# paninski-lab/lightning-pose

Hardware: AMD Instinct MI355X
Metric: training frames/sec (whole node), ResNet-50 384x384 17-kp semi-sup (higher is better)
Workload: dtype bf16; 1 GPU; C2/C3: ResNet-50 SemiSupervisedHeatmapTracker 384x384, K=17, 64 labeled + 128 unlabeled frames per GPU, heatmap_mse + temporal + pca_singleview + unimodal_mse, Adam (backbone lr=0 as at step 0), bf16-mixed; global_batch=192, parallelism=dp1, sync_batchnorm=False, decode_prune=plain kernels (chosen from the maps)

## Files before the change

### include/lp_hip.h

```cpp
#ifndef LP_HIP_H
#define LP_HIP_H

#include <stddef.h>
#include <stdint.h>

#ifdef __cplusplus
extern "C" {
#endif

typedef void* lp_stream_t;

int lp_config_reload_env(void);

enum {
    LP_OK = 0,
    LP_ERR_ARGUMENT = -1,
    LP_ERR_UNSUPPORTED = -2,
};

enum { LP_TF_NONE = 0, LP_TF_SINGLE = 1, LP_TF_PER_FRAME = 2, LP_TF_PER_VIEW = 3 };

#define LP_HIP_ABI_VERSION 153
int lp_version(void);
const char* lp_strerror(int code);


typedef struct lp_decode_tables {
    const int* row_base;
    const float* row_taps;
    const int* col_start;
    const float* col_taps;
    const int* colT_start;
    const float* colT_taps;
    int ty, tx, tc;
} lp_decode_tables;

typedef struct lp_frame_map {
// ... 80 lines not shown
    int B, Hi, Wi, Ci;
    int Ho, Wo, Co;
    int R, S, stride, pad;
} lp_conv_geom;

#define LP_CONV_KERNEL_IGEMM 0
#define LP_CONV_KERNEL_PIPE 1
#define LP_CONV_KERNEL_WGRAD 2
#define LP_CONV_KERNEL_WGRAD_PIPE 3
#define LP_CONV_KERNEL_PIPE_HALO 4
#define LP_CONV_KERNEL_STEM_WGRAD_NB 8
#define LP_CONV_KERNEL_WGRAD_NB 9
#define LP_CONV_KERNEL_RES2D 5
int lp_conv_last_kernel(void);
int lp_conv_last_resident(void);

int lp_conv_fwd(const void* x, const void* w, const lp_conv_geom* geom, const float* bias, void* out_bf16, float* out_f32, int ldo,
                int n_store, lp_stream_t stream);
int lp_conv_dgrad(const void* dy, const void* wd, const lp_conv_geom* geom, const float* bias, const void* addend,
                  const void* relu_mask, void* dx_bf16, float* dx_f32, int ldo, int n_store, int skip_empty_classes,
                  lp_stream_t stream);
typedef struct lp_gemm_batch {
    int nb, nh;
    long long a_b, a_h, b_b, b_h, c_b, c_h;
} lp_gemm_batch;
int lp_gemm_nt(const void* a, int lda, const void* b, int ldb, void* c_bf16, float* c_f32, int ldc, int M, int N, int K, int n_store,
               const float* bias, const lp_gemm_batch* batch, lp_stream_t stream);
int lp_gemm_tn(const void* x, int ldx, const void* y, int ldy, void* out_bf16, int ldo, int M, int J, int N, const lp_gemm_batch* batch,
               lp_stream_t stream);
int lp_attn_fwd(const void* qkv_bf16, int ld_qkv, int k_off, int v_off, int B, int nh, int T, float scale, void* p_bf16, int ldp,
// ... 304 lines not shown
```

### lightning-pose_amd/_lib.py

```python

from __future__ import annotations

import ctypes as C
import os

_HERE = os.path.dirname(os.path.abspath(__file__))
LIB_PATH = os.environ.get("LP_HIP_LIB") or os.path.join(_HERE, "liblp_hip.so")


class LpHipUnavailable(RuntimeError):
    """liblp_hip.so could not be loaded, or an op was given a non-ROCm tensor.  There is no fallback path."""


class LpHipError(RuntimeError):
    pass


class DecodeTables(C.Structure):
    _fields_ = [("row_base", C.c_void_p), ("row_taps", C.c_void_p), ("col_start", C.c_void_p),
                ("col_taps", C.c_void_p), ("colT_start", C.c_void_p), ("colT_taps", C.c_void_p),
                ("ty", C.c_int), ("tx", C.c_int), ("tc", C.c_int)]


class FrameMap(C.Structure):
# ... 34 lines not shown
CONV_KERNEL_LABEL = {
    CONV_KERNEL_PIPE: (("conv_igemm_kernel", "conv_pipe_kernel"),),
    CONV_KERNEL_PIPE_HALO: (("conv_igemm_kernel", "conv_pipe_kernel"), (">", ",halo>")),
    CONV_KERNEL_RES2D: (("conv_igemm_kernel<64,", "conv_res2d_kernel<"), ("conv_igemm_kernel<64>", "conv_res2d_kernel<fwd>")),
    CONV_KERNEL_WGRAD_PIPE: (("conv_wgrad_kernel", "conv_wgrad_pipe_kernel"),),
    CONV_KERNEL_WGRAD_NB: (("conv_wgrad_kernel", "conv_wgrad_nb_kernel"),),
}
BORDER_RENORM, BORDER_CLAMP = 0, 1
AUG_GEOM, AUG_BLUR, AUG_DROPOUT, AUG_DROP_PER_CHANNEL, AUG_SALT, AUG_PEPPER = 1, 2, 4, 8, 16, 32
AUG_ELASTIC, AUG_HISTEQ, AUG_CLAHE, AUG_EMBOSS, AUG_CROPPAD, AUG_HFLIP = 64, 128, 256, 512, 1024, 2048
AUG_OP_DROPOUT, AUG_OP_SALT, AUG_OP_PEPPER, AUG_OP_ELASTIC = 0, 1, 2, 3
AUG_LOCAL_BLUR_COARSE, AUG_LOCAL_EMBOSS = 0, 1
AUG_ELASTIC_MAX_RADIUS = 20
TF_NONE, TF_SINGLE, TF_PER_FRAME, TF_PER_VIEW = 0, 1, 2, 3

ABI_VERSION = 153

_P, _I, _F, _L, _Z = C.c_void_p, C.c_int, C.c_float, C.c_long, C.c_size_t

PROTOTYPES = {
    "lp_version": (_I, []),
    "lp_strerror": (C.c_char_p, [_I]),
    "lp_config_reload_env": (_I, []),
    "lp_decode_window": (_I, [_I, _I]),
    "lp_decode_fwd": (_I, [_P, _I, _I, _I, _I, _I, _F, C.POINTER(DecodeTables), C.POINTER(FrameMap), _P, _P, _P, _P, _I, _P]),
    "lp_decode_bwd": (_I, [_P, _I, _I, _I, _I, _I, _F, C.POINTER(DecodeTables), C.POINTER(FrameMap), _P, _P, _P, _P, _I, _I, _P]),
    "lp_frame_map_apply": (_I, [_P, _I, _I, C.POINTER(FrameMap), _I, _P, _P]),
    "lp_heatmap_gen": (_I, [_P, _P, _I, _I, _I, _I, _I, _I, _F, _P, _P]),
    "lp_heatmap_gen_bwd": (_I, [_P, _P, _I, _I, _I, _I, _I, _I, _F, _P, _P, _P]),
    "lp_temporal_heatmap_workspace_bytes": (_Z, [_I, _I]),
    "lp_temporal_heatmap_fwd": (_I, [_I, _P, _P, _I, _I, _I, _I, _P, _F, _P, _P, _P]),
# ... 16 lines not shown
    "lp_kp_metrics": (_I, [_P, _P, _I, _I, C.POINTER(PcaSpec), C.POINTER(PcaSpec), _P, _P, _P, _P, _P]),
    "lp_conv_fwd": (_I, [_P, _P, C.POINTER(ConvGeom), _P, _P, _P, _I, _I, _P]),
    "lp_conv_dgrad": (_I, [_P, _P, C.POINTER(ConvGeom), _P, _P, _P, _P, _P, _I, _I, _I, _P]),
    "lp_conv_dgrad_bits": (_I, [_P, _P, C.POINTER(ConvGeom), _P, _P, _P, _I, _P]),
    "lp_gemm_nt": (_I, [_P, _I, _P, _I, _P, _P, _I, _I, _I, _I, _I, _P, C.POINTER(GemmBatch), _P]),
    "lp_gemm_nt_gelu_bwd": (_I, [_P, _P, _P, _P, _I, _I, _I, _P, _P]),
    "lp_gemm_nt_gelu_fwd": (_I, [_P, _P, _P, _P, _P, _I, _I, _I, _P]),
    "lp_gemm_tn": (_I, [_P, _I, _P, _I, _P, _I, _I, _I, _I, C.POINTER(GemmBatch), _P]),
    "lp_attn_fwd": (_I, [_P, _I, _I, _I, _I, _I, _I, C.c_float, _P, _I, _P, _I, _P]),
    "lp_attn_bwd_kv": (_I, [_P, _I, _I, _P, _I, _P, _I, _P, _I, _I, _I, C.c_float, _P, _P, _I, _I, _I, _P]),
    "lp_attn_rowdot": (_I, [_P, _P, _I, _I, _I, _P, _P]),
    "lp_attn_dscores": (_I, [_P, _I, _P, _I, _P, _P, _I, C.c_longlong, C.c_longlong, C.c_float, _P, _I, _I, _I, _I, C.POINTER(GemmBatch), _P]),
    "lp_conv_fwd_bn": (_I, [_P, _P, C.POINTER(ConvGeom), _P, C.POINTER(BnFuse), _P]),
    "lp_conv_last_kernel": (_I, []),
    "lp_conv_last_resident": (_I, []),
    "lp_stem_fwd_bn": (_I, [_P, _P, C.POINTER(ConvGeom), _P, C.POINTER(BnFuse), _P]),
    "lp_conv_dgrad_bn": (_I, [_P, _P, C.POINTER(ConvGeom), _P, _P, _P, C.POINTER(BnFuse), _P]),
    "lp_bn_fold": (_I, [_P, _P, _P, _P, _P, _F, _I, _I, _P, _P, _P]),
    "lp_conv_fwd_act": (_I, [_P, _P, C.POINTER(ConvGeom), _P, _P, _I, _P, _P]),
    "lp_conv_wgrad_workspace_bytes": (_Z, [C.POINTER(ConvGeom), _I]),
    "lp_conv_wgrad": (_I, [_P, _P, C.POINTER(ConvGeom), _P, _I, _P, _Z, _P]),
    "lp_conv_wgrad_bias": (_I, [_P, _P, C.POINTER(ConvGeom), _P, _P, _I, _P, C.c_size_t, _P]),
    "lp_stem_fwd": (_I, [_P, _P, C.POINTER(ConvGeom), _P, _P]),
    "lp_stem_wgrad": (_I, [_P, _P, C.POINTER(ConvGeom), _P, _I, _P, _Z, _P]),
    "lp_bn_reduce_workspace_bytes": (_Z, [_I, _I]),
    "lp_bn_stats": (_I, [_P, _I, _I, _P, _P, _Z, _P]),
    "lp_bn_finalize": (_I, [_P, _F, _I, _F, _F, _P, _P, _P, _P, _P]),
    "lp_fxsum_accumulate": (_I, [_P, _I, _P, _P]),
    "lp_bn_finalize_f32": (_I, [_P, _F, _I, _F, _F, _P, _P, _P, _P, _P]),
    "lp_bn_finalize2": (_I, [_P, _F, _F, _I, _F, _F, _P, _P, _P, _P, _P]),
# ... 156 lines not shown
```

### lightning-pose_amd/csrc/api.hip

```cpp
#include "lp_common.h"

#include <stdlib.h>

#include <atomic>

extern "C" int lp_version(void) { return LP_HIP_ABI_VERSION; }

namespace lp {
static int env_int(const char* name, int dflt) {
    const char* e = getenv(name);
    return (e == nullptr || *e == 0) ? dflt : atoi(e);
}
static LpSwitches read_switches() {
    LpSwitches s;
    s.conv_pipe = env_int("LP_CONV_PIPE", 1);
    s.conv_halo = env_int("LP_CONV_HALO", 1);
    s.pipe_wres = env_int("LP_PIPE_WRES", 1);
    s.conv_res2d = env_int("LP_CONV_RES2D", 1);
    s.infer_pipe = env_int("LP_INFER_PIPE", 1);
    s.gemm_pipe = env_int("LP_GEMM_PIPE", 1);
    s.wgrad_pipe = env_int("LP_WGRAD_PIPE", 1);
    s.wgrad_nb = env_int("LP_WGRAD_NB", 1);
    s.stem_2d = env_int("LP_STEM_2D", 1);
    s.stem_wgrad_nb = env_int("LP_STEM_WGRAD_NB", 1);
    s.pool_v2 = env_int("LP_POOL_V2", 1);
    s.bn_bwd_wgs_per_cu = env_int("LP_BN_BWD_WGS_PER_CU", 5);
    if (s.bn_bwd_wgs_per_cu < 1 || s.bn_bwd_wgs_per_cu > 5) s.bn_bwd_wgs_per_cu = 5;
    s.conv_max_wgs = env_int("LP_CONV_MAX_WGS", 0);
    return s;
}
static std::atomic<const LpSwitches*> g_switches{new LpSwitches(read_switches())};
const LpSwitches& lp_switches() { return *g_switches.load(std::memory_order_acquire); }
}

extern "C" int lp_config_reload_env(void) {
    lp::g_switches.store(new lp::LpSwitches(lp::read_switches()), std::memory_order_release);
    return LP_OK;
// ... 10 lines not shown
```

### lightning-pose_amd/csrc/conv.hip

```cpp
#include <stdlib.h>

#include "lp_common.h"

namespace lp {

constexpr int kBM = 128;
constexpr int kBK = 64;
constexpr int kLD = kBK + 8;

struct ConvGeom {
    int B, Hi, Wi, Ci;
    int Ho, Wo, Co;
    int R, S, stride, pad;
};

struct ConvEpilogue {
    unsigned short* out_bf16;
    float* out_f32;
    int ldo;
    int n_store;
    const float* bias;
    const unsigned short* addend;
    const unsigned short* relu_mask;
    const unsigned char* relu_bits;
// ... 908 lines not shown
}

static long long seg_split_rows(int seg_images, int B, long long rows_per_image, long long M) {
    if (seg_images <= 0) return M;
    if (seg_images >= B) return -1;
    const long long r = (long long)seg_images * rows_per_image;
    return (r % kBM == 0) ? r : -1;
}

static void bn_fuse_begin(ConvEpilogue& ep, const lp_bn_fuse* bn) {
    ep.stats_sums = bn->sums;
    ep.seg_images = bn->seg_images;
}

static thread_local int g_last_conv_kernel = LP_CONV_KERNEL_IGEMM;
static thread_local int g_last_conv_resident = 0;

struct ConvRoute {
    int kernel;
    int bn;
    int mode;
    int ek;
    bool wres;
};
constexpr int kNoKernel = -1;

struct ConvProblem {
    int mode;
    int ek;
    const void *x, *w;
// ... 231 lines not shown
    const long long b_elems = (z.nb - 1) * z.b_b + (z.nh - 1) * z.b_h + (long long)(N - 1) * ldb + K;
    const long long c_elems = (z.nb - 1) * z.c_b + (z.nh - 1) * z.c_h + (long long)M * ldc;
    if (a_elems >= (1LL << 31) || b_elems >= (1LL << 31) || c_elems >= (1LL << 32)) return LP_ERR_UNSUPPORTED;
    if ((z.a_b | z.a_h | z.b_b | z.b_h) % 8 != 0 || (z.c_b | z.c_h) % c_align != 0) return LP_ERR_UNSUPPORTED;
    p = conv_problem(mode, a, b, ConvGeom{1, 1, M, K, 1, M, N, 1, 1, 1, 0}, 1, M, N, K);
    p.dense = z.nb * z.nh == 1 && lda == K && ldb == K && ldc == N;
    p.gemm = true, p.nz = z.nb * z.nh, p.x_bytes = (unsigned)(2 * a_elems), p.w_bytes = (unsigned)(2 * b_elems);
    p.gx = GemmExt{lda, ldb, z.nh, 0, (unsigned)(2 * z.a_b), (unsigned)(2 * z.a_h), (unsigned)(2 * z.b_b), (unsigned)(2 * z.b_h), (unsigned)z.c_b,
                   (unsigned)z.c_h};
    return LP_OK;
}

}
#include "conv_stem_wgrad.h"
#include "conv_wgrad_nb.h"
namespace lp {

constexpr int kWgradWgs = 512;

struct WgradRoute {
    bool ok;
    int kernel;
    int split, per;
    size_t ws_floats;
    int bn, tiles_a, tiles_b;
    bool swap, tuned;
    int Ka, Cb;
    int kh, PT, lead;
};

static void slice_pixels(WgradRoute& p, int units, int ksteps, int split, int cap) {
    if (split > cap) split = cap;
    if (split < 1) split = 1;
    p.per = ((ksteps + split - 1) / split) * kBK;
    p.split = (units + p.per - 1) / p.per;
}

static WgradRoute plan_wgrad(int M, int Kw, int Co, int split_hint) {
    WgradRoute p{};
    p.kernel = LP_CONV_KERNEL_WGRAD;
    p.bn = Co > 64 ? 128 : 64;
    p.tiles_a = (Kw + kBM - 1) / kBM;
    p.tiles_b = p.bn == 128 ? (Co + 127) / 128 : 1;
    const int tiles = p.tiles_a * p.tiles_b, ksteps = (M + kBK - 1) / kBK;
    slice_pixels(p, M, ksteps, split_hint > 0 ? split_hint : kWgradWgs / tiles, ksteps < 65535 ? ksteps : 65535);
    p.ws_floats = (size_t)p.split * tiles * 4 * 2 * (p.bn / 64) * 16 * 64;
    p.ok = true;
    return p;
}

// ... 32 lines not shown
    if (split <= 0) {
        double best = 1e30;
        for (int s = 1; s <= 2 * cus && s <= ksteps / 2; ++s) {
            if (s != 1 && (tiles * s) % cus > 0 && (tiles * (s + 1) + cus - 1) / cus == (tiles * s + cus - 1) / cus) continue;
            const double rounds = (double)((tiles * s + cus - 1) / cus), per = (double)((ksteps + s - 1) / s);
            const double cost = rounds * per + 0.04 * (p.bn / 128.0) * s * tiles + 2.0 * rounds;
            if (cost < best) best = cost, split = s;
        }
    }
    slice_pixels(p, M, ksteps, split, ksteps / 2);
    p.ws_floats = (size_t)p.split * tiles * 256 * p.bn;
    p.ok = true;
    return p;
}

static WgradRoute plan_wgrad_nb(const ConvGeom& g, int split_hint) {
    WgradRoute p{};
    if (g.R != 3 || g.S != 3 || g.stride != 1 || g.pad != 1 || g.Hi != g.Ho || g.Wi != g.Wo || g.Ci % 64 != 0 || g.Co % 64 != 0) return p;
    if (g.Wi > 126) return p;
    const long long pt = (long long)g.B * (g.Hi + 1) * (g.Wi + 1);
    if (pt + 64 * 8 >= (1LL << 31)) return p;
    p.kernel = LP_CONV_KERNEL_WGRAD_NB;
    p.PT = (int)pt;
    p.lead = 1 + (g.Wi + 1) / 64;
    p.bn = g.Co % 128 == 0 ? 128 : 64;
    p.kh = p.bn == 64 ? 2 : 1;
    p.tiles_a = g.Ci / 64;
    p.tiles_b = g.Co / p.bn;
    const int tiles = p.tiles_a * p.tiles_b;
    const int ksteps = (p.PT + kBK - 1) / kBK;
// ... 6 lines not shown
            const double rounds = (double)((tiles * s + cus - 1) / cus), per = (double)((ksteps + s - 1) / s);
            const double cost = rounds * (per * step_us + 15.0) + 0.06 * s * tiles;
            if (cost < best) best = cost, split = s;
        }
    }
    slice_pixels(p, p.PT, ksteps, split, ksteps < 65535 ? ksteps : 65535);
    p.ws_floats = (size_t)p.split * p.kh * tiles * 9 * 64 * p.bn;
    p.ok = true;
    return p;
}

static bool is_stem(const ConvGeom& g) { return g.R == 7 && g.S == 7 && g.stride == 2 && g.pad == 3 && g.Ci == 4 && g.Co == 64; }

struct WgradCandidates {
    int n;
    WgradRoute r[3];
};

static WgradCandidates wgrad_candidates(const ConvGeom& g, bool stem, int split_hint) {
    WgradCandidates c{};
    const int M = g.B * g.Ho * g.Wo;
    auto add = [&c](const WgradRoute& p) {
        if (p.ok) c.r[c.n++] = p;
    };
    if (stem) {
        if (lp_switches().stem_wgrad_nb != 0) add(plan_stem_wgrad_nb(g, split_hint));
        add(plan_wgrad(M, 256, 64, split_hint));
    } else {
        add(plan_wgrad_nb(g, split_hint));
        add(plan_wgrad_pipe(g, split_hint));
        add(plan_wgrad(M, g.R * g.S * g.Ci, g.Co, split_hint));
    }
    return c;
}

static const WgradRoute& route_wgrad(const WgradCandidates& c, const LpSwitches& sw, bool dbias) {
    const bool pipe = !dbias && sw.conv_pipe != 0;
    for (int i = 0; i < c.n - 1; ++i) {
        const WgradRoute& r = c.r[i];
        if (r.kernel == LP_CONV_KERNEL_WGRAD_NB && !(pipe && sw.wgrad_pipe == 1 && sw.wgrad_nb != 0)) continue;
        if (r.kernel == LP_CONV_KERNEL_WGRAD_PIPE && !(pipe && sw.wgrad_pipe != 0 && (sw.wgrad_pipe == 2 || r.tuned))) continue;
        return r;
    }
    return c.r[c.n - 1];
}

template <int BN>
static void launch_wgrad(const WgradRoute& p, const void* x, const void* dy, const ConvGeom& g, float* dw, float* dbias, float* ws, hipStream_t st) {
    const int M = g.B * g.Ho * g.Wo, Kw = g.R * g.S * g.Ci, tiles = p.tiles_a * p.tiles_b;
    const unsigned x_bytes = (unsigned)(2ull * g.B * g.Hi * g.Wi * g.Ci), dy_bytes = (unsigned)(2ull * M * g.Co);
    TnExt ext{};
    ext.col_sums = dbias;
    const auto kernel = dbias ? conv_wgrad_kernel<BN, false, true> : conv_wgrad_kernel<BN, false, false>;
    hipLaunchKernelGGL(kernel, dim3(tiles * p.split), dim3(256), 0, st, (const unsigned short*)x, (const unsigned short*)dy, x_bytes, dy_bytes, g,
                       M, Kw, tiles, p.tiles_b, p.per, make_fastdiv(g.Ho * g.Wo), make_fastdiv(g.Wo), ws, ext);
    launch_wgrad_reduce<BN>(ws, p.split, tiles, p.tiles_b, Kw, g.Co, dw, st);
// ... 7 lines not shown
    const void *pa = x, *qb = dy;
    unsigned pa_bytes = x_bytes, qb_bytes = dy_bytes;
    if (p.swap) {
        wg = WgradPipeGeom{g.B, g.Ho, g.Wo, g.Ho, g.Wo, g.Co, 1, 1, 1, 0, p.Ka, p.Cb, 1};
        pa = dy, qb = x, pa_bytes = dy_bytes, qb_bytes = x_bytes;
    } else {
        const int plain = g.R == 1 && g.S == 1 && g.stride == 1 && g.pad == 0 && g.Hi == g.Ho && g.Wi == g.Wo;
        wg = WgradPipeGeom{g.B, g.Hi, g.Wi, g.Ho, g.Wo, g.Ci, g.R, g.S, g.stride, g.pad, p.Ka, p.Cb, plain};
    }
    const int tiles = p.tiles_a * p.tiles_b;
    const int sa = p.swap ? Kw : 1, sb = p.swap ? 1 : Kw;
    hipLaunchKernelGGL((conv_wgrad_pipe_kernel<BN>), dim3(tiles * p.split), dim3(512), 0, st, (const unsigned short*)pa, (const unsigned short*)qb,
                       pa_bytes, qb_bytes, wg, M, tiles, p.tiles_b, p.per, make_fastdiv(g.Ho * g.Wo), make_fastdiv(g.Wo), ws);
    hipLaunchKernelGGL((wgrad_pipe_reduce_kernel<BN>), dim3(tiles * 256 * BN / 64), dim3(256), 0, st, ws, p.split, tiles, p.tiles_b, p.Ka, p.Cb,
                       sa, sb, dw);
}

template <int BN>
static void launch_wgrad_nb(const WgradRoute& p, const void* x, const void* dy, const ConvGeom& g, float* dw, float* ws, hipStream_t st) {
    const unsigned x_bytes = (unsigned)(2ull * g.B * g.Hi * g.Wi * g.Ci), dy_bytes = (unsigned)(2ull * g.B * g.Ho * g.Wo * g.Co);
    const WgradNbGeom ng{g.B, g.Hi, g.Wi, g.Ci, g.Co, p.PT, p.lead};
    const int tiles = p.tiles_a * p.tiles_b;
    hipLaunchKernelGGL((conv_wgrad_nb_kernel<BN>), dim3(tiles * p.split), dim3(512), 0, st, (const unsigned short*)x, (const unsigned short*)dy,
                       x_bytes, dy_bytes, ng, tiles, p.tiles_b, p.per, make_fastdiv(g.Wi + 1), make_fastdiv(g.Hi + 1), ws);
    hipLaunchKernelGGL((wgrad_nb_reduce_kernel<BN>), dim3(tiles * 9 * BN), dim3(256), 0, st, ws, p.split * p.kh, tiles, p.tiles_b, g.Ci, dw);
}

static bool geom_ok(const lp_conv_geom* c) {
    return c && c->B > 0 && c->Hi > 0 && c->Wi > 0 && c->Ci > 0 && c->Ho > 0 && c->Wo > 0 && c->Co > 0 && c->R > 0 && c->S > 0 &&
           c->stride > 0 && c->pad >= 0;
// ... 17 lines not shown
    ConvProblem p = conv_problem(kModeFwd, x, w, g, g.Ho, g.Wo, g.Co, g.R * g.S * g.Ci);
    p.ek = kEkNone;
    p.ep = ConvEpilogue{(unsigned short*)out_bf16, out_f32, ldo, n_store > 0 ? n_store : p.N, bias};
    if (bn) {
        LP_REQUIRE(bn->sums && bn->seg_images >= 0);
        if (p.N % 8 != 0) return LP_ERR_UNSUPPORTED;
        p.seg_rows = seg_split_rows(bn->seg_images, g.B, (long long)g.Ho * g.Wo, p.M);
        if (p.seg_rows < 0) return LP_ERR_UNSUPPORTED;
        bn_fuse_begin(p.ep, bn);
    }
    return run_conv(p, stream);
}

extern "C" int lp_conv_last_kernel(void) { return lp::g_last_conv_kernel; }
extern "C" int lp_conv_last_resident(void) { return lp::g_last_conv_resident; }

extern "C" int lp_conv_fwd(const void* x, const void* w, const lp_conv_geom* geom, const float* bias, void* out_bf16, float* out_f32,
                           int ldo, int n_store, lp_stream_t stream) {
    return conv_fwd_impl(x, w, geom, bias, out_bf16, out_f32, ldo, n_store, nullptr, stream);
}

extern "C" int lp_conv_fwd_act(const void* x, const void* w, const lp_conv_geom* geom, const float* bias, const void* residual_bf16, int relu,
                               void* out_bf16, lp_stream_t stream) {
    using namespace lp;
    LP_REQUIRE(x && w && geom_ok(geom) && out_bf16);
    ConvGeom g = to_geom(geom);
    if (g.Ci % kBK != 0 || g.Co % 8 != 0 || g.R * g.S > 32 || (long long)g.B * g.Hi * g.Wi * g.Ci >= (1LL << 31) ||
        (long long)g.B * g.Ho * g.Wo * g.Co >= (1LL << 32))
        return LP_ERR_UNSUPPORTED;
    ConvProblem p = conv_problem(kModeInfer, x, w, g, g.Ho, g.Wo, g.Co, g.R * g.S * g.Ci);
// ... 175 lines not shown
static int conv_wgrad_impl(const void* x, const void* dy, const lp_conv_geom* geom, float* dw, float* dbias, int split_hint, void* workspace,
                           size_t workspace_bytes, lp_stream_t stream) {
    using namespace lp;
    LP_REQUIRE(x && dy && geom_ok(geom) && dw && workspace);
    ConvGeom g = to_geom(geom);
    if (g.Ci % 8 != 0 || g.Co % 8 != 0 || (long long)g.B * g.Hi * g.Wi * g.Ci >= (1LL << 31) ||
        (long long)g.B * g.Ho * g.Wo * g.Co >= (1LL << 31))
        return LP_ERR_UNSUPPORTED;
    const WgradCandidates c = wgrad_candidates(g, false, split_hint);
    const WgradRoute& p = route_wgrad(c, lp_switches(), dbias != nullptr);
    LP_REQUIRE(workspace_bytes >= p.ws_floats * sizeof(float));
    hipStream_t st = (hipStream_t)stream;
    float* ws = (float*)workspace;
    g_last_conv_kernel = p.kernel;
    g_last_conv_resident = 0;
    if (p.kernel == LP_CONV_KERNEL_WGRAD_NB) {
        if (p.bn == 128) launch_wgrad_nb<128>(p, x, dy, g, dw, ws, st);
        else launch_wgrad_nb<64>(p, x, dy, g, dw, ws, st);
    } else if (p.kernel == LP_CONV_KERNEL_WGRAD_PIPE) {
        if (p.bn == 128) launch_wgrad_pipe<128>(p, x, dy, g, dw, ws, st);
        else launch_wgrad_pipe<64>(p, x, dy, g, dw, ws, st);
    } else {
        if (p.bn == 128) launch_wgrad<128>(p, x, dy, g, dw, dbias, ws, st);
        else launch_wgrad<64>(p, x, dy, g, dw, dbias, ws, st);
    }
    return launch_status();
}

extern "C" int lp_conv_wgrad(const void* x, const void* dy, const lp_conv_geom* geom, float* dw, int split_hint, void* workspace,
                             size_t workspace_bytes, lp_stream_t stream) {
    return conv_wgrad_impl(x, dy, geom, dw, nullptr, split_hint, workspace, workspace_bytes, stream);
}

extern "C" int lp_conv_wgrad_bias(const void* x, const void* dy, const lp_conv_geom* geom, float* dw, float* dbias, int split_hint,
                                  void* workspace, size_t workspace_bytes, lp_stream_t stream) {
// ... 68 lines not shown
                             size_t workspace_bytes, lp_stream_t stream) {
    using namespace lp;
    LP_REQUIRE(x4 && dy && geom_ok(geom) && dw && workspace);
    ConvGeom g = to_geom(geom);
    if (!is_stem(g)) return LP_ERR_UNSUPPORTED;
    const WgradCandidates c = wgrad_candidates(g, true, split_hint);
    const WgradRoute& p = route_wgrad(c, lp_switches(), false);
    LP_REQUIRE(workspace_bytes >= p.ws_floats * sizeof(float));
    const int M = g.B * g.Ho * g.Wo, Kw = 256;
    const unsigned short *xs = (const unsigned short*)x4, *dys = (const unsigned short*)dy;
    const FastDiv dhw = make_fastdiv(g.Ho * g.Wo), dwo = make_fastdiv(g.Wo);
    hipStream_t st = (hipStream_t)stream;
    float* ws = (float*)workspace;
    g_last_conv_kernel = p.kernel;
    g_last_conv_resident = 0;
    if (p.kernel == LP_CONV_KERNEL_STEM_WGRAD_NB)
        hipLaunchKernelGGL(stem_wgrad_nb_kernel, dim3(p.split), dim3(256), 0, st, xs, dys, (unsigned)(8ull * g.B * g.Hi * g.Wi),
                           (unsigned)(128ull * M), g, M, p.per, dhw, dwo, ws);
    else
        hipLaunchKernelGGL((conv_wgrad_kernel<64, true>), dim3(p.tiles_a * p.split), dim3(256), 0, st, xs, dys, 0u, 0u, g, M, Kw, p.tiles_a, 1,
                           p.per, dhw, dwo, ws, TnExt{});
    launch_wgrad_reduce<64>(ws, p.split, p.tiles_a, 1, Kw, 64, dw, st);
    return launch_status();
}
```

### lightning-pose_amd/csrc/lp_common.h

```cpp
#pragma once

#include <hip/hip_runtime.h>
#include <stdint.h>

#include "../../include/lp_hip.h"

namespace lp {

constexpr int kWave = 64;

typedef __attribute__((ext_vector_type(8))) __bf16 bf16x8;
typedef __attribute__((ext_vector_type(8))) unsigned short u16x8;
typedef __attribute__((ext_vector_type(4))) unsigned short u16x4;
typedef __attribute__((ext_vector_type(4))) float f32x4;
typedef __attribute__((ext_vector_type(16))) float f32x16;

__device__ __forceinline__ float bf16_to_f32(unsigned short b) { return __uint_as_float(((unsigned)b) << 16); }

#if defined(__HIP_DEVICE_COMPILE__)
typedef __attribute__((ext_vector_type(2))) __bf16 bf16x2_t;
typedef __attribute__((ext_vector_type(2))) float f32x2_t;
__device__ __forceinline__ unsigned short f32_to_bf16(float f) { return __builtin_bit_cast(unsigned short, (__bf16)f); }
__device__ __forceinline__ unsigned pack_bf16x2(float lo, float hi) {
    const f32x2_t v = {lo, hi};
// ... 232 lines not shown
    }
    td = fmin(fmax(td, -0x1p49), 0x1p49);
    const double h = rint(td * 0x1p12);
    const long long hi = (long long)h;
    const long long lo = (long long)rint((td - h * 0x1p-12) * 0x1p60);
    atomicAdd(reinterpret_cast<unsigned long long*>(&p->hi), (unsigned long long)hi);
    atomicAdd(reinterpret_cast<unsigned long long*>(&p->lo), (unsigned long long)lo);
}
__device__ __forceinline__ float fx_value(const lp_fxsum* p) {
    const long long lo = p->lo;
    if (lo >= kFxPoisonSeen || lo <= -kFxPoisonSeen) return __int_as_float(0x7fc00000);
    return (float)((double)p->hi * 0x1p-12 + (double)lo * 0x1p-60);
}

struct LpSwitches {
    int conv_pipe, conv_halo, pipe_wres, conv_res2d, infer_pipe, gemm_pipe, wgrad_pipe, wgrad_nb, stem_2d, stem_wgrad_nb, pool_v2, conv_max_wgs, bn_bwd_wgs_per_cu;
};
const LpSwitches& lp_switches();

inline int launch_status() {
    hipError_t e = hipGetLastError();
    return e == hipSuccess ? LP_OK : (int)e;
}

}

#define LP_REQUIRE(cond)                    \
    do {                                    \
        if (!(cond)) return LP_ERR_ARGUMENT; \
    } while (0)
```

### lightning-pose_amd/engine.py

```python

from __future__ import annotations

import ctypes as C
import math
import os
from dataclasses import dataclass, field

import torch
import torch.distributed as dist

from . import _lib
from ._lib import check
from . import ops
from .ops import _p

BN_EPS = 1e-5
BN_MOMENTUM = 0.1
CPAD = 64


@dataclass
class ConvP:
    name: str
    kind: str
# ... 227 lines not shown
        return torch.zeros(n, device=self.device, dtype=torch.float32)

    def _zeros_fx(self, n: int) -> torch.Tensor:
        return self._zeros_f32(4 * n).view(torch.int64)

    def _timed(self, tag: str, flops: float, fn, nbytes: float = 0.0, layer: str = ""):
        if self.profile is None:
            return fn()
        e0, e1 = torch.cuda.Event(enable_timing=True), torch.cuda.Event(enable_timing=True)
        e0.record()
        out = fn()
        e1.record()
        if tag.startswith("conv_") and hasattr(self._lib, "lp_conv_last_kernel"):
            for old, new in _lib.CONV_KERNEL_LABEL.get(self._lib.lp_conv_last_kernel(), ()):
                tag = tag.replace(old, new)
        self.profile.append((tag, flops, e0, e1, nbytes, layer))
        return out

    def _wgrad(self, x, dy, g, dw: torch.Tensor, stem: bool = False, dbias: torch.Tensor | None = None) -> None:
        need = self._lib.lp_conv_wgrad_workspace_bytes(C.byref(g), 0)
        if self._wgrad_ws is None or self._wgrad_ws.numel() < need:
            self._join_side_stream()
            self._wgrad_ws = torch.empty(max(need, 96 << 20), device=self.device, dtype=torch.uint8)
        fn = self._lib.lp_stem_wgrad if stem else self._lib.lp_conv_wgrad
        what = "lp_stem_wgrad" if stem else "lp_conv_wgrad"
        if dbias is not None:
            what = "lp_conv_wgrad_bias"
            fn = lambda x_, dy_, g_, dw_, split, ws, nws, st: self._lib.lp_conv_wgrad_bias(x_, dy_, g_, dw_, _p(dbias), split, ws, nws, st)
        if self.device.type != "cuda" or not self.wgrad_side_stream or self.profile is not None:
            check(fn(_p(x), _p(dy), C.byref(g), _p(dw), 0, _p(self._wgrad_ws), self._wgrad_ws.numel(), ops._stream()), what)
# ... 709 lines not shown
```

### profiles/kernel_resources.py

```python
import os
import re
import shutil
import subprocess
import sys
import tempfile

ROOT = os.path.dirname(os.path.dirname(os.path.abspath(__file__)))
LLVM = os.path.join(os.environ.get("ROCM_PATH", "/opt/rocm"), "lib", "llvm", "bin")
HOT = ("lp::conv_pipe_kernel", "lp::conv_spec_kernel", "lp::conv_wgrad_pipe_kernel", "lp::conv_res2d_kernel", "lp::conv_stem2d_kernel", "lp::conv_wgrad_kernel", "lp::stem_wgrad_nb_kernel", "lp::conv_wgrad_nb_kernel",
       "lp::conv_igemm_kernel", "lp::bn_apply_kernel", "lp::bn_bwd_apply_kernel", "lp::bn_relu_maxpool_fwd_kernel", "lp::bn_pool_bwd_v2_kernel",
       "lp::colreduce_kernel", "lp::rows_reduce_kernel", "lp::decode_fwd_kernel", "lp::decode_bwd_kernel", "lp::heatmap_gen_kernel",
       "lp::hm_rowsq_kernel", "lp::hm_grad_kernel", "lp::softmax2d", "lp::adam_kernel", "lp::pca_kernel", "lp::temporal_kernel",
       "lp::attn_fwd_kernel", "lp::attn_bwd_kv_kernel", "lp::pixel_shuffle",
       "lp::layernorm_ls_fwd_kernel", "lp::layernorm_ls_bwd_kernel",
       "lp::rope_kernel", "lp::vit_reg_tokens_fwd_kernel", "lp::vit_reg_tokens_bwd_kernel",
       "lp::window_partition_kernel", "lp::window_unpartition_kernel", "lp::vit_pos_tokens_fwd_kernel", "lp::vit_pos_tokens_bwd_kernel",
       "lp::resid_out_fwd_kernel", "lp::resid_out_bwd_kernel",
       "lp::frames_crop_resize_kernel", "lp::bbox_from_keypoints_kernel", "lp::bbox_smooth_kernel")
ALLOWED_SCRATCH = (
    re.compile(r"lp::decode_bwd_kernel<\d+, \d+, 64, "),
    re.compile(r"lp::bn_bwd_apply_kernel<false, false>"),
    re.compile(r"lp::conv_igemm_kernel<128, 1>"),
)

# ... 48 lines not shown
```

Measured before the change: 4851 frames/s.

## Add 256x256-tile wide wgrad kernel for large 1x1 and strided convs

```diff
diff --git a/include/lp_hip.h b/include/lp_hip.h
--- a/include/lp_hip.h
+++ b/include/lp_hip.h
@@ -20,7 +20,7 @@
 
 enum { LP_TF_NONE = 0, LP_TF_SINGLE = 1, LP_TF_PER_FRAME = 2, LP_TF_PER_VIEW = 3 };
 
-#define LP_HIP_ABI_VERSION 153
+#define LP_HIP_ABI_VERSION 154
 int lp_version(void);
 const char* lp_strerror(int code);
 
@@ -131,6 +131,7 @@
 #define LP_CONV_KERNEL_RES2D 5
 int lp_conv_last_kernel(void);
 int lp_conv_last_resident(void);
+int lp_conv_last_wgrad_tile(void);
 
 int lp_conv_fwd(const void* x, const void* w, const lp_conv_geom* geom, const float* bias, void* out_bf16, float* out_f32, int ldo,
                 int n_store, lp_stream_t stream);
diff --git a/lightning-pose_amd/_lib.py b/lightning-pose_amd/_lib.py
--- a/lightning-pose_amd/_lib.py
+++ b/lightning-pose_amd/_lib.py
@@ -72,7 +72,7 @@
 AUG_ELASTIC_MAX_RADIUS = 20
 TF_NONE, TF_SINGLE, TF_PER_FRAME, TF_PER_VIEW = 0, 1, 2, 3
 
-ABI_VERSION = 153
+ABI_VERSION = 154
 
 _P, _I, _F, _L, _Z = C.c_void_p, C.c_int, C.c_float, C.c_long, C.c_size_t
 
@@ -119,6 +119,7 @@
     "lp_conv_fwd_bn": (_I, [_P, _P, C.POINTER(ConvGeom), _P, C.POINTER(BnFuse), _P]),
     "lp_conv_last_kernel": (_I, []),
     "lp_conv_last_resident": (_I, []),
+    "lp_conv_last_wgrad_tile": (_I, []),
     "lp_stem_fwd_bn": (_I, [_P, _P, C.POINTER(ConvGeom), _P, C.POINTER(BnFuse), _P]),
     "lp_conv_dgrad_bn": (_I, [_P, _P, C.POINTER(ConvGeom), _P, _P, _P, C.POINTER(BnFuse), _P]),
     "lp_bn_fold": (_I, [_P, _P, _P, _P, _P, _F, _I, _I, _P, _P, _P]),
diff --git a/lightning-pose_amd/csrc/api.hip b/lightning-pose_amd/csrc/api.hip
--- a/lightning-pose_amd/csrc/api.hip
+++ b/lightning-pose_amd/csrc/api.hip
@@ -21,6 +21,7 @@
     s.gemm_pipe = env_int("LP_GEMM_PIPE", 1);
     s.wgrad_pipe = env_int("LP_WGRAD_PIPE", 1);
     s.wgrad_nb = env_int("LP_WGRAD_NB", 1);
+    s.wgrad_wide = env_int("LP_WGRAD_WIDE", 1);
     s.stem_2d = env_int("LP_STEM_2D", 1);
     s.stem_wgrad_nb = env_int("LP_STEM_WGRAD_NB", 1);
     s.pool_v2 = env_int("LP_POOL_V2", 1);
diff --git a/lightning-pose_amd/csrc/conv.hip b/lightning-pose_amd/csrc/conv.hip
--- a/lightning-pose_amd/csrc/conv.hip
+++ b/lightning-pose_amd/csrc/conv.hip
@@ -946,6 +946,7 @@
 }
 
 static thread_local int g_last_conv_kernel = LP_CONV_KERNEL_IGEMM;
+static thread_local int g_last_wgrad_tile = 0;
 static thread_local int g_last_conv_resident = 0;
 
 struct ConvRoute {
@@ -1207,6 +1208,7 @@
 }
 #include "conv_stem_wgrad.h"
 #include "conv_wgrad_nb.h"
+#include "conv_wgrad_wide.h"
 namespace lp {
 
 constexpr int kWgradWgs = 512;
@@ -1227,6 +1229,12 @@
     if (split < 1) split = 1;
     p.per = ((ksteps + split - 1) / split) * kBK;
     p.split = (units + p.per - 1) / p.per;
+}
+
+static bool wgrad_wide_tuned(const ConvGeom& g, bool one, int Ka, int Cb) {
+    if (!one && g.stride != 2) return false;
+    if ((long long)Ka * Cb >= 220LL * (Ka + Cb)) return true;
+    return one && Ka == 256 && Cb == 1024;
 }
 
 static WgradRoute plan_wgrad(int M, int Kw, int Co, int split_hint) {
@@ -1289,6 +1297,40 @@
     return p;
 }
 
+static WgradRoute plan_wgrad_wide(const ConvGeom& g, int split_hint, int mode) {
+    WgradRoute p{};
+    const int M = g.B * g.Ho * g.Wo, Kw = g.R * g.S * g.Ci;
+    const bool one = g.R == 1 && g.S == 1 && g.stride == 1 && g.pad == 0 && g.Hi == g.Ho && g.Wi == g.Wo;
+    if (g.Ci % 8 != 0 || g.Co % 64 != 0 || M < kWideBK) return p;
+    const bool can = g.Co % 256 == 0, can_swap = one && Kw % 256 == 0;
+    if (!can && !can_swap) return p;
+    p.kernel = LP_CONV_KERNEL_WGRAD_PIPE;
+    p.bn = 256;
+    p.swap = can_swap && (!can || mode == 3);
+    p.Ka = p.swap ? g.Co : Kw;
+    p.Cb = p.swap ? Kw : g.Co;
+    p.tiles_a = (p.Ka + 255) / 256;
+    p.tiles_b = p.Cb / 256;
+    if ((long long)p.tiles_a * 256 * 8 > (long long)p.Ka * 9) return p;
+    p.tuned = wgrad_wide_tuned(g, one, p.Ka, p.Cb);
+    const int tiles = p.tiles_a * p.tiles_b;
+    const int cus = conv_max_wgs(1);
+    const int ksteps = (M + kBK - 1) / kBK;
+    int split = split_hint;
+    if (split <= 0) {
+        double best = 1e30;
+        for (int s = 1; s <= 2 * cus && s <= ksteps / 2; ++s) {
+            const double rounds = (double)((tiles * s + cus - 1) / cus), per = (double)((ksteps + s - 1) / s);
+            const double cost = rounds * (per * 0.85 + 1.3) + 0.13 * s * tiles;
+            if (cost < best) best = cost, split = s;
+        }
+    }
+    slice_pixels(p, M, ksteps, split, ksteps / 2);
+    p.ws_floats = (size_t)p.split * tiles * 256 * 256;
+    p.ok = true;
+    return p;
+}
+
 static WgradRoute plan_wgrad_nb(const ConvGeom& g, int split_hint) {
     WgradRoute p{};
     if (g.R != 3 || g.S != 3 || g.stride != 1 || g.pad != 1 || g.Hi != g.Ho || g.Wi != g.Wo || g.Ci % 64 != 0 || g.Co % 64 != 0) return p;
@@ -1325,7 +1367,7 @@
 
 struct WgradCandidates {
     int n;
-    WgradRoute r[3];
+    WgradRoute r[4];
 };
 
 static WgradCandidates wgrad_candidates(const ConvGeom& g, bool stem, int split_hint) {
@@ -1339,6 +1381,7 @@
         add(plan_wgrad(M, 256, 64, split_hint));
     } else {
         add(plan_wgrad_nb(g, split_hint));
+        if (lp_switches().wgrad_wide != 0) add(plan_wgrad_wide(g, split_hint, lp_switches().wgrad_wide));
         add(plan_wgrad_pipe(g, split_hint));
         add(plan_wgrad(M, g.R * g.S * g.Ci, g.Co, split_hint));
     }
@@ -1350,7 +1393,8 @@
     for (int i = 0; i < c.n - 1; ++i) {
         const WgradRoute& r = c.r[i];
         if (r.kernel == LP_CONV_KERNEL_WGRAD_NB && !(pipe && sw.wgrad_pipe == 1 && sw.wgrad_nb != 0)) continue;
-        if (r.kernel == LP_CONV_KERNEL_WGRAD_PIPE && !(pipe && sw.wgrad_pipe != 0 && (sw.wgrad_pipe == 2 || r.tuned))) continue;
+        if (r.kernel == LP_CONV_KERNEL_WGRAD_PIPE && r.bn == 256 && !(pipe && sw.wgrad_pipe != 0 && (sw.wgrad_wide >= 2 || (sw.wgrad_pipe == 1 && r.tuned)))) continue;
+        if (r.kernel == LP_CONV_KERNEL_WGRAD_PIPE && r.bn != 256 && !(pipe && sw.wgrad_pipe != 0 && (sw.wgrad_pipe == 2 || r.tuned))) continue;
         return r;
     }
     return c.r[c.n - 1];
@@ -1388,6 +1432,28 @@
                        pa_bytes, qb_bytes, wg, M, tiles, p.tiles_b, p.per, make_fastdiv(g.Ho * g.Wo), make_fastdiv(g.Wo), ws);
     hipLaunchKernelGGL((wgrad_pipe_reduce_kernel<BN>), dim3(tiles * 256 * BN / 64), dim3(256), 0, st, ws, p.split, tiles, p.tiles_b, p.Ka, p.Cb,
                        sa, sb, dw);
+}
+
+static void launch_wgrad_wide(const WgradRoute& p, const void* x, const void* dy, const ConvGeom& g, float* dw, float* ws, hipStream_t st) {
+    const int M = g.B * g.Ho * g.Wo, Kw = g.R * g.S * g.Ci;
+    const unsigned x_bytes = (unsigned)(2ull * g.B * g.Hi * g.Wi * g.Ci), dy_bytes = (unsigned)(2ull * M * g.Co);
+    WgradPipeGeom wg{};
+    const void *pa = x, *qb = dy;
+    unsigned pa_bytes = x_bytes, qb_bytes = dy_bytes;
+    if (p.swap) {
+        wg = WgradPipeGeom{g.B, g.Ho, g.Wo, g.Ho, g.Wo, g.Co, 1, 1, 1, 0, p.Ka, p.Cb, 1};
+        pa = dy, qb = x, pa_bytes = dy_bytes, qb_bytes = x_bytes;
+    } else {
+        const int plain = g.R == 1 && g.S == 1 && g.stride == 1 && g.pad == 0 && g.Hi == g.Ho && g.Wi == g.Wo;
+        wg = WgradPipeGeom{g.B, g.Hi, g.Wi, g.Ho, g.Wo, g.Ci, g.R, g.S, g.stride, g.pad, p.Ka, p.Cb, plain};
+    }
+    const int tiles = p.tiles_a * p.tiles_b;
+    const int sa = p.swap ? Kw : 1, sb = p.swap ? 1 : Kw;
+    const auto kernel = p.swap ? conv_wgrad_wide_kernel<false> : conv_wgrad_wide_kernel<true>;
+    const auto reduce = p.swap ? wgrad_wide_reduce_kernel<false> : wgrad_wide_reduce_kernel<true>;
+    hipLaunchKernelGGL(kernel, dim3(tiles * p.split), dim3(512), 0, st, (const unsigned short*)pa, (const unsigned short*)qb, pa_bytes, qb_bytes,
+                       wg, M, tiles, p.tiles_b, p.per, make_fastdiv(g.Ho * g.Wo), make_fastdiv(g.Wo), ws);
+    hipLaunchKernelGGL(reduce, dim3(tiles * 256 * 4), dim3(256), 0, st, ws, p.split, tiles, p.tiles_b, p.Ka, p.Cb, sa, sb, dw);
 }
 
 template <int BN>
@@ -1435,6 +1501,7 @@
 
 extern "C" int lp_conv_last_kernel(void) { return lp::g_last_conv_kernel; }
 extern "C" int lp_conv_last_resident(void) { return lp::g_last_conv_resident; }
+extern "C" int lp_conv_last_wgrad_tile(void) { return lp::g_last_wgrad_tile; }
 
 extern "C" int lp_conv_fwd(const void* x, const void* w, const lp_conv_geom* geom, const float* bias, void* out_bf16, float* out_f32,
                            int ldo, int n_store, lp_stream_t stream) {
@@ -1640,11 +1707,13 @@
     float* ws = (float*)workspace;
     g_last_conv_kernel = p.kernel;
     g_last_conv_resident = 0;
+    g_last_wgrad_tile = p.kernel == LP_CONV_KERNEL_WGRAD_PIPE ? p.bn : 0;
     if (p.kernel == LP_CONV_KERNEL_WGRAD_NB) {
         if (p.bn == 128) launch_wgrad_nb<128>(p, x, dy, g, dw, ws, st);
         else launch_wgrad_nb<64>(p, x, dy, g, dw, ws, st);
     } else if (p.kernel == LP_CONV_KERNEL_WGRAD_PIPE) {
-        if (p.bn == 128) launch_wgrad_pipe<128>(p, x, dy, g, dw, ws, st);
+        if (p.bn == 256) launch_wgrad_wide(p, x, dy, g, dw, ws, st);
+        else if (p.bn == 128) launch_wgrad_pipe<128>(p, x, dy, g, dw, ws, st);
         else launch_wgrad_pipe<64>(p, x, dy, g, dw, ws, st);
     } else {
         if (p.bn == 128) launch_wgrad<128>(p, x, dy, g, dw, dbias, ws, st);
@@ -1743,6 +1812,7 @@
     float* ws = (float*)workspace;
     g_last_conv_kernel = p.kernel;
     g_last_conv_resident = 0;
+    g_last_wgrad_tile = 0;
     if (p.kernel == LP_CONV_KERNEL_STEM_WGRAD_NB)
         hipLaunchKernelGGL(stem_wgrad_nb_kernel, dim3(p.split), dim3(256), 0, st, xs, dys, (unsigned)(8ull * g.B * g.Hi * g.Wi),
                            (unsigned)(128ull * M), g, M, p.per, dhw, dwo, ws);
diff --git a/lightning-pose_amd/csrc/conv_wgrad_wide.h b/lightning-pose_amd/csrc/conv_wgrad_wide.h
--- /dev/null
+++ b/lightning-pose_amd/csrc/conv_wgrad_wide.h
@@ -0,0 +1,206 @@
+#pragma once
+
+namespace lp {
+
+constexpr int kWideBK = 32, kWideStages = 4;
+
+template <bool TR>
+__global__ __launch_bounds__(512) void conv_wgrad_wide_kernel(const unsigned short* __restrict__ Pa, const unsigned short* __restrict__ Qb,
+                                                              unsigned pa_bytes, unsigned qb_bytes, WgradPipeGeom g, int M, int tiles,
+                                                              int tiles_b, int m_per_split, FastDiv div_hw, FastDiv div_wo,
+                                                              float* __restrict__ ws) {
+    constexpr int NT = 4;
+    constexpr int kRow = 512;
+    constexpr int kStageA = kWideBK * kRow, kStage = 2 * kStageA;
+    __shared__ __attribute__((aligned(16))) unsigned char smem[kWideStages * kStage];
+
+    const int tid = threadIdx.x, lane = tid & 63;
+    const int wave = __builtin_amdgcn_readfirstlane(tid >> 6);
+    const int wm = wave & 3, wn = wave >> 2;
+    const int work = xcd_remap(blockIdx.x, gridDim.x);
+    const int slice = work / tiles, tile = work - slice * tiles;
+    const int a0 = (tile / tiles_b) * 256, b0 = (tile % tiles_b) * 256;
+    const int m_begin = slice * m_per_split, m_end = min(M, m_begin + m_per_split);
+    const int KT = (m_end - m_begin + kWideBK - 1) / kWideBK;
+    const buf_rsrc rsrc_a = make_buf_rsrc(Pa, pa_bytes), rsrc_b = make_buf_rsrc(Qb, qb_bytes);
+    unsigned long long dst_bits = (unsigned long long)(ws + ((((size_t)slice * tiles + tile) * 8 + wave) * (2 * 4 * 16)) * 64 + lane);
+    LP_OPAQUE(dst_bits);
+
+    const int lrow = wave * 2 + (lane >> 5);
+    const int lchunk = (lane & 31) ^ ((lrow & 3) << 2);
+    const int ja = a0 + lchunk * 8;
+    const bool ja_ok = ja < g.Ka;
+    const int tap = (ja_ok ? ja : 0) / g.Ca;
+    const int tcn = (ja_ok ? ja : 0) - tap * g.Ca;
+    const int tr = tap / g.S, ts = tap - tr * g.S;
+    const unsigned boff = (unsigned)(b0 + lchunk * 8) * 2u;
+    const int hw = g.Ho * g.Wo;
+
+    unsigned is_a[2], is_b[2];
+    unsigned char* is_dst = smem;
+    auto prep_step = [&](int st, int kt) {
+        const int mk = m_begin + kt * kWideBK;
+#pragma unroll
+        for (int p = 0; p < 2; ++p) {
+            const int m = mk + p * 16 + lrow;
+            const bool in = m < m_end && kt < KT;
+            bool ok = in && ja_ok;
+            unsigned off;
+            if (g.plain) {
+                off = (unsigned)(m * g.Ca + tcn) * 2u;
+            } else {
+                const int mm = ok ? m : 0;
+                const int b = fdiv(mm, div_hw), rem = mm - b * hw;
+                const int ho = fdiv(rem, div_wo), wo = rem - ho * g.Wo;
+                const int hi = ho * g.stride - g.pad + tr, wi = wo * g.stride - g.pad + ts;
+                ok = ok && hi >= 0 && hi < g.Hi && wi >= 0 && wi < g.Wi;
+                off = (unsigned)(((b * g.Hi + hi) * g.Wi + wi) * g.Ca + tcn) * 2u;
+            }
+            is_a[p] = ok ? off : ~0u;
+            is_b[p] = in ? (unsigned)m * (unsigned)(g.Cb * 2) + boff : ~0u;
+        }
+        is_dst = smem + st * kStage;
+    };
+    auto issue_load = [&](int i) {
+        if (i < 2) buf_load16_lds(rsrc_a, is_dst + (i * 16 + wave * 2) * kRow, is_a[i], 0u);
+        else buf_load16_lds(rsrc_b, is_dst + kStageA + ((i - 2) * 16 + wave * 2) * kRow, is_b[i - 2], 0u);
+    };
+
+    const int fq = lane >> 4, fi = lane & 15;
+    const int frow = (fq >> 1) * 8 + (fi >> 2), fcol = (fq & 1) * 16 + (fi & 3) * 4;
+    const int sw = (frow & 3) << 2;
+    unsigned foa[2], fob[NT];
+#pragma unroll
+    for (int mt = 0; mt < 2; ++mt) {
+        const int e0 = wm * 64 + mt * 32 + fcol;
+        foa[mt] = (unsigned)(frow * kRow + (((e0 >> 3) ^ sw) << 4) + (e0 & 7) * 2);
+    }
+#pragma unroll
+    for (int nt = 0; nt < NT; ++nt) {
+        const int e0 = wn * 128 + nt * 32 + fcol;
+        fob[nt] = (unsigned)(kStageA + frow * kRow + (((e0 >> 3) ^ sw) << 4) + (e0 & 7) * 2);
+    }
+    f32x16 acc[2][NT];
+#pragma unroll
+    for (int mt = 0; mt < 2; ++mt)
+#pragma unroll
+        for (int nt = 0; nt < NT; ++nt)
+#pragma unroll
+            for (int e = 0; e < 16; ++e) acc[mt][nt][e] = 0.f;
+
+    bf16x8 a[2][2], b[2][NT];
+    auto fetch = [&](int st, auto kk_c) {
+        constexpr int kk = decltype(kk_c)::value;
+        typedef __attribute__((ext_vector_type(8))) short s16x8_t;
+        const unsigned char* sb = smem + st * kStage;
+#pragma unroll
+        for (int mt = 0; mt < 2; ++mt) {
+            const s16x4_t lo = lds_read_tr16_async_off<kk * 16 * kRow>(sb + foa[mt]), hi = lds_read_tr16_async_off<kk * 16 * kRow + 4 * kRow>(sb + foa[mt]);
+            const s16x8_t v = {lo[0], lo[1], lo[2], lo[3], hi[0], hi[1], hi[2], hi[3]};
+            a[kk][mt] = __builtin_bit_cast(bf16x8, v);
+        }
+#pragma unroll
+        for (int nt = 0; nt < NT; ++nt) {
+            const s16x4_t lo = lds_read_tr16_async_off<kk * 16 * kRow>(sb + fob[nt]), hi = lds_read_tr16_async_off<kk * 16 * kRow + 4 * kRow>(sb + fob[nt]);
+            const s16x8_t v = {lo[0], lo[1], lo[2], lo[3], hi[0], hi[1], hi[2], hi[3]};
+            b[kk][nt] = __builtin_bit_cast(bf16x8, v);
+        }
+    };
+    auto mma = [&](auto kk_c) {
+        constexpr int kk = decltype(kk_c)::value;
+#pragma unroll
+        for (int mt = 0; mt < 2; ++mt)
+#pragma unroll
+            for (int nt = 0; nt < NT; ++nt)
+                acc[mt][nt] = TR ? __builtin_amdgcn_mfma_f32_32x32x16_bf16(b[kk][nt], a[kk][mt], acc[mt][nt], 0, 0, 0)
+                                 : __builtin_amdgcn_mfma_f32_32x32x16_bf16(a[kk][mt], b[kk][nt], acc[mt][nt], 0, 0, 0);
+    };
+    const std::integral_constant<int, 0> k0{};
+    const std::integral_constant<int, 1> k1{};
+
+#pragma unroll
+    for (int s = 0; s < 3; ++s) {
+        prep_step(s, s);
+#pragma unroll
+        for (int i = 0; i < 4; ++i) issue_load(i);
+    }
+    auto first_half = [&](int cur, int kt) {
+        prep_step(cur == 0 ? kWideStages - 1 : cur - 1, kt + 3);
+        fetch(cur, k1);
+        __builtin_amdgcn_sched_barrier(0);
+        LP_WAIT_LGKM_TOUCH4(12, a[0][0], a[0][1], b[0][0], b[0][1]);
+        LP_WAIT_LGKM_TOUCH3(12, b[0][2], b[0][3], a[0][0]);
+        mma(k0);
+        issue_load(0);
+        issue_load(1);
+        __builtin_amdgcn_sched_barrier(0);
+        LP_WAIT_LGKM_TOUCH4(0, a[1][0], a[1][1], b[1][0], b[1][1]);
+        LP_WAIT_LGKM_TOUCH3(0, b[1][2], b[1][3], a[1][0]);
+    };
+    LP_WAIT_VM(8);
+    LP_RAW_BARRIER();
+    fetch(0, k0);
+    first_half(0, 0);
+    int cur = 0;
+    for (int kt = 1; kt < KT; ++kt) {
+        const int nxt = cur == kWideStages - 1 ? 0 : cur + 1;
+        LP_WAIT_VM(6);
+        LP_RAW_BARRIER();
+        fetch(nxt, k0);
+        __builtin_amdgcn_sched_barrier(0);
+        mma(k1);
+        issue_load(2);
+        issue_load(3);
+        __builtin_amdgcn_sched_barrier(0);
+        first_half(nxt, kt);
+        cur = nxt;
+    }
+    mma(k1);
+    LP_WAIT_VM(0);
+    float* dst = reinterpret_cast<float*>(dst_bits);
+#pragma unroll
+    for (int mt = 0; mt < 2; ++mt)
+#pragma unroll
+        for (int nt = 0; nt < NT; ++nt)
+#pragma unroll
+            for (int e = 0; e < 16; ++e) dst[((mt * NT + nt) * 16 + e) * 64] = acc[mt][nt][e];
+}
+
+template <bool TR>
+__global__ __launch_bounds__(256) void wgrad_wide_reduce_kernel(const float* __restrict__ ws, int slices, int tiles, int tiles_b, int Ka, int Cb,
+                                                                int sa, int sb, float* __restrict__ dW) {
+    constexpr int NT = 4;
+    constexpr int PER_TILE = 8 * 2 * NT * 16 * 64;
+    __shared__ float part[4][64];
+    const size_t total = (size_t)tiles * PER_TILE;
+    const int lane = threadIdx.x & 63, w = threadIdx.x >> 6;
+    const size_t i = (size_t)blockIdx.x * 64 + lane;
+    float s0 = 0.f, s1 = 0.f;
+    int sl = w;
+    for (; sl + 4 < slices; sl += 8) {
+        s0 += ws[(size_t)sl * total + i];
+        s1 += ws[(size_t)(sl + 4) * total + i];
+    }
+    for (; sl < slices; sl += 4) s0 += ws[(size_t)sl * total + i];
+    part[w][lane] = s0 + s1;
+    __syncthreads();
+    if (w == 0) {
+        const float sum = (part[0][lane] + part[1][lane]) + (part[2][lane] + part[3][lane]);
+        size_t t = i >> 6;
+        const int e = (int)(t & 15);
+        t >>= 4;
+        const int nt = (int)(t % NT);
+        t /= NT;
+        const int mt = (int)(t & 1);
+        t >>= 1;
+        const int wave = (int)(t & 7);
+        const int tile = (int)(t >> 3);
+        const int wm = wave & 3, wn = wave >> 2;
+        const int row = (e & 3) + 8 * (e >> 2) + 4 * (lane >> 5), col = lane & 31;
+        const int a = (tile / tiles_b) * 256 + wm * 64 + mt * 32 + (TR ? col : row);
+        const int b = (tile % tiles_b) * 256 + wn * 128 + nt * 32 + (TR ? row : col);
+        if (a < Ka && b < Cb) dW[(size_t)a * sa + (size_t)b * sb] += sum;
+    }
+}
+
+}
diff --git a/lightning-pose_amd/csrc/lp_common.h b/lightning-pose_amd/csrc/lp_common.h
--- a/lightning-pose_amd/csrc/lp_common.h
+++ b/lightning-pose_amd/csrc/lp_common.h
@@ -270,7 +270,7 @@
 }
 
 struct LpSwitches {
-    int conv_pipe, conv_halo, pipe_wres, conv_res2d, infer_pipe, gemm_pipe, wgrad_pipe, wgrad_nb, stem_2d, stem_wgrad_nb, pool_v2, conv_max_wgs, bn_bwd_wgs_per_cu;
+    int conv_pipe, conv_halo, pipe_wres, conv_res2d, infer_pipe, gemm_pipe, wgrad_pipe, wgrad_nb, wgrad_wide, stem_2d, stem_wgrad_nb, pool_v2, conv_max_wgs, bn_bwd_wgs_per_cu;
 };
 const LpSwitches& lp_switches();
 
diff --git a/lightning-pose_amd/engine.py b/lightning-pose_amd/engine.py
--- a/lightning-pose_amd/engine.py
+++ b/lightning-pose_amd/engine.py
@@ -265,6 +265,8 @@
         if tag.startswith("conv_") and hasattr(self._lib, "lp_conv_last_kernel"):
             for old, new in _lib.CONV_KERNEL_LABEL.get(self._lib.lp_conv_last_kernel(), ()):
                 tag = tag.replace(old, new)
+            if tag.startswith("conv_wgrad_pipe_kernel") and self._lib.lp_conv_last_wgrad_tile() == 256:
+                tag = "conv_wgrad_wide_kernel" + tag[tag.index(">") + 1:]
         self.profile.append((tag, flops, e0, e1, nbytes, layer))
         return out
 
diff --git a/profiles/kernel_resources.py b/profiles/kernel_resources.py
--- a/profiles/kernel_resources.py
+++ b/profiles/kernel_resources.py
@@ -7,7 +7,7 @@
 
 ROOT = os.path.dirname(os.path.dirname(os.path.abspath(__file__)))
 LLVM = os.path.join(os.environ.get("ROCM_PATH", "/opt/rocm"), "lib", "llvm", "bin")
-HOT = ("lp::conv_pipe_kernel", "lp::conv_spec_kernel", "lp::conv_wgrad_pipe_kernel", "lp::conv_res2d_kernel", "lp::conv_stem2d_kernel", "lp::conv_wgrad_kernel", "lp::stem_wgrad_nb_kernel", "lp::conv_wgrad_nb_kernel",
+HOT = ("lp::conv_pipe_kernel", "lp::conv_spec_kernel", "lp::conv_wgrad_pipe_kernel", "lp::conv_res2d_kernel", "lp::conv_stem2d_kernel", "lp::conv_wgrad_kernel", "lp::stem_wgrad_nb_kernel", "lp::conv_wgrad_nb_kernel", "lp::conv_wgrad_wide_kernel",
        "lp::conv_igemm_kernel", "lp::bn_apply_kernel", "lp::bn_bwd_apply_kernel", "lp::bn_relu_maxpool_fwd_kernel", "lp::bn_pool_bwd_v2_kernel",
        "lp::colreduce_kernel", "lp::rows_reduce_kernel", "lp::decode_fwd_kernel", "lp::decode_bwd_kernel", "lp::heatmap_gen_kernel",
        "lp::hm_rowsq_kernel", "lp::hm_grad_kernel", "lp::softmax2d", "lp::adam_kernel", "lp::pca_kernel", "lp::temporal_kernel",
```

Result: no change. 4893 frames/s, median of 6 (+0.9%).
